# cloudflare/zkp-ecdsa

Measured on NVIDIA H100. Metric: ZKAttest proofs/sec, higher is better.
Workload: dtype u256/u258 (32-bit limbs, Montgomery)

## Files before the change

### zkp_ecdsa_b200/csrc/zk_ops.cuh

```cuda
#pragma once
#include "zk_curves.cuh"
#include "zk_layout.h"
#include "zk_sha256.cuh"

namespace zk {

#if defined(__CUDA_ARCH__)
#define ZK_SET_STATUS(ptr, code) atomicCAS((int*)(ptr), 0, (int)(code))
#define ZK_SET_STATUS_OVER(ptr, code, over) \
  do {                                      \
    atomicCAS((int*)(ptr), 0, (int)(code)); \
    atomicCAS((int*)(ptr), (int)(over), (int)(code)); \
  } while (0)
#else
#define ZK_SET_STATUS_OVER(ptr, code, over)              \
  do {                                                   \
    if (*(ptr) == 0 || *(ptr) == (over)) *(ptr) = (code); \
  } while (0)
#define ZK_SET_STATUS(ptr, code) \
  do {                           \
    if (*(ptr) == 0) *(ptr) = (code); \
  } while (0)
#endif

template <int N>
ZK_HD void ld(uint32_t* r, const uint32_t* p) {
#pragma unroll
  for (int i = 0; i < N; i++) r[i] = p[i];
}
template <int N>
ZK_HD void st(uint32_t* p, const uint32_t* r) {
#pragma unroll
  for (int i = 0; i < N; i++) p[i] = r[i];
}

enum : int {
  P256_PROJ_WORDS = 24,
  P256_AFF_WORDS = 16,
#if defined(ZKA_PG_WAR256)
  TOM_PROJ_WORDS = 24,
  TOM_E2_WORDS = 24,
  TOM_AFF_WORDS = 16,
  TOM_PRE_WORDS = 16,
#else
  TOM_PROJ_WORDS = 28,
  TOM_E2_WORDS = 36,
  TOM_AFF_WORDS = 18,
  TOM_PRE_WORDS = 32,
#endif
  NORM_CHUNK_MAX = 64,
};


#if defined(ZKA_PG_WAR256)
ZK_HD void tom_st_xyz(uint32_t* m, const uint32_t* x, const uint32_t* y, const uint32_t* z) {
  st<8>(m, x); st<8>(m + 8, y); st<8>(m + 16, z);
}
ZK_HD void tom_ld_xyz(uint32_t* x, uint32_t* y, uint32_t* z, const uint32_t* m) {
  ld<8>(x, m); ld<8>(y, m + 8); ld<8>(z, m + 16);
}
ZK_HD void tom_ld_pre(TomPre& q, const uint32_t* m) { ld<8>(q.x, m); ld<8>(q.y, m + 8); }
#else
ZK_HD void tom_st_xyz(uint32_t* m, const uint32_t* x, const uint32_t* y, const uint32_t* z) {
  uint32_t w[28];
#pragma unroll
  for (int i = 0; i < 9; i++) { w[i] = x[i]; w[9 + i] = y[i]; w[18 + i] = z[i]; }
  w[27] = 0;
#if defined(__CUDA_ARCH__)
  uint4* v = reinterpret_cast<uint4*>(m);
#pragma unroll
  for (int i = 0; i < 7; i++) v[i] = make_uint4(w[4 * i], w[4 * i + 1], w[4 * i + 2], w[4 * i + 3]);
#else
  for (int i = 0; i < 28; i++) m[i] = w[i];
#endif
}
ZK_HD void tom_ld_xyz(uint32_t* x, uint32_t* y, uint32_t* z, const uint32_t* m) {
  uint32_t w[28];
#if defined(__CUDA_ARCH__)
  const uint4* v = reinterpret_cast<const uint4*>(m);
#pragma unroll
  for (int i = 0; i < 7; i++) {
    const uint4 u = v[i];
    w[4 * i] = u.x; w[4 * i + 1] = u.y; w[4 * i + 2] = u.z; w[4 * i + 3] = u.w;
  }
#else
  for (int i = 0; i < 28; i++) w[i] = m[i];
#endif
#pragma unroll
  for (int i = 0; i < 9; i++) { x[i] = w[i]; y[i] = w[9 + i]; z[i] = w[18 + i]; }
}
ZK_HD void tom_st_efgh(uint32_t* m, const TomEfgh& p) {
  uint32_t w[36];
#pragma unroll
  for (int i = 0; i < 9; i++) { w[i] = p.e[i]; w[9 + i] = p.f[i]; w[18 + i] = p.g[i]; w[27 + i] = p.h[i]; }
#if defined(__CUDA_ARCH__)
  uint4* v = reinterpret_cast<uint4*>(m);
#pragma unroll
  for (int i = 0; i < 9; i++) v[i] = make_uint4(w[4 * i], w[4 * i + 1], w[4 * i + 2], w[4 * i + 3]);
#else
  for (int i = 0; i < 36; i++) m[i] = w[i];
#endif
}
ZK_HD void tom_ld_efgh(uint32_t* e, uint32_t* f, uint32_t* g, uint32_t* h, const uint32_t* m) {
  uint32_t w[36];
#if defined(__CUDA_ARCH__)
  const uint4* v = reinterpret_cast<const uint4*>(m);
#pragma unroll
  for (int i = 0; i < 9; i++) {
    const uint4 u = v[i];
    w[4 * i] = u.x; w[4 * i + 1] = u.y; w[4 * i + 2] = u.z; w[4 * i + 3] = u.w;
  }
#else
  for (int i = 0; i < 36; i++) w[i] = m[i];
#endif
#pragma unroll
  for (int i = 0; i < 9; i++) { e[i] = w[i]; f[i] = w[9 + i]; g[i] = w[18 + i]; h[i] = w[27 + i]; }
}

ZK_HD void tom2_pre_neg(TomPre& q, bool neg) {
  uint32_t nk[9];
  Tomp::neg(nk, q.k);
#pragma unroll
  for (int i = 0; i < 9; i++) {
    const uint32_t a = q.x[i], b = q.y[i];
    q.x[i] = neg ? b : a;
    q.y[i] = neg ? a : b;
    q.k[i] = neg ? nk[i] : q.k[i];
  }
}
ZK_HD void tom_ld_pre(TomPre& q, const uint32_t* m) {
#if defined(__CUDA_ARCH__)
  const uint4* v = reinterpret_cast<const uint4*>(m);
  uint32_t w[32];
#pragma unroll
  for (int i = 0; i < 7; i++) {
    uint4 u = __ldg(v + i);
    w[4 * i] = u.x; w[4 * i + 1] = u.y; w[4 * i + 2] = u.z; w[4 * i + 3] = u.w;
  }
#pragma unroll
  for (int i = 0; i < 9; i++) { q.x[i] = w[i]; q.y[i] = w[9 + i]; q.k[i] = w[18 + i]; }
#else
  ld<9>(q.x, m); ld<9>(q.y, m + 9); ld<9>(q.k, m + 18);
#endif
}

#endif

ZK_HD void ld4(uint32_t* w, const void* p) {
#if defined(__CUDA_ARCH__)
  const uint4 u = *reinterpret_cast<const uint4*>(p);
  w[0] = u.x; w[1] = u.y; w[2] = u.z; w[3] = u.w;
#else
  const uint32_t* q = reinterpret_cast<const uint32_t*>(p);
  for (int i = 0; i < 4; i++) w[i] = q[i];
#endif
}
ZK_HD void st4(void* p, const uint32_t* w) {
#if defined(__CUDA_ARCH__)
  *reinterpret_cast<uint4*>(p) = make_uint4(w[0], w[1], w[2], w[3]);
#else
  uint32_t* q = reinterpret_cast<uint32_t*>(p);
  for (int i = 0; i < 4; i++) q[i] = w[i];
#endif
}
ZK_HD void ld8v(uint32_t* r, const uint32_t* p) { ld4(r, p); ld4(r + 4, p + 4); }
ZK_HD void st8v(uint32_t* p, const uint32_t* r) { st4(p, r); st4(p + 4, r + 4); }
ZK_HD bool aligned16(const void* p) { return ((size_t)p & 15) == 0; }

template <int N, int CB>
// ... 245 lines not shown
      const uint32_t* src = proj + (size_t)(lo + k) * TOM_PROJ_WORDS;
      uint32_t xx[9];
      tom_ld_xyz(xx, y, z, src);
      F::mul(den, y, z);
      F::mul(acc, acc, den);
      copy_n<9>(pf[k], acc);
    }
    uint32_t inv[9], s2[9], dd2[9];
    F::inv(inv, acc);
    tom_const(s2, TOM_SQRTND1);
    tom_const(dd2, TOM_2D2);
    for (int k = n - 1; k >= 0; k--) {
      const uint32_t* src = proj + (size_t)(lo + k) * TOM_PROJ_WORDS;
      uint32_t x[9], di[9], w[9], v[9], kk[9], ym[9], yp[9];
      tom_ld_xyz(x, y, z, src);
      F::mul(den, y, z);
      if (k > 0) F::mul(di, inv, pf[k - 1]); else copy_n<9>(di, inv);
      F::mul(inv, inv, den);
      F::mul(w, x, y);
      F::mul(w, w, di);
      F::mul(w, w, s2);
      F::sqr(v, z);
      F::mul(v, v, di);
      F::mul(kk, w, v);
      F::mul(kk, kk, dd2);
      F::sub(ym, v, w);
      F::add(yp, v, w);
      F::reduce(ym); F::reduce(yp); F::reduce(kk);
      uint32_t* o = pre + (size_t)(lo + k) * TOM_PRE_WORDS;
      st<9>(o, ym); st<9>(o + 9, yp); st<9>(o + 18, kk);
      for (int i = 27; i < 32; i++) o[i] = 0;
    }
  }
};

struct TomNormTask {
  const uint32_t* proj;
  uint32_t* aff;
  uint8_t* bytes;
  int count;
  int chunk;
  int e2;
  int aff_mod, aff_lim;
  int stride;
  ZK_HD static void canon2p(uint32_t* r) {
    uint32_t t[9], p2[9];
#pragma unroll
    for (int i = 0; i < 9; i++) p2[i] = (FpTom::p(i) << 1) | (i > 0 ? (FpTom::p(i - 1) >> 31) : 0u);
    uint32_t br = sub_n<9>(t, r, p2);
    csel_n<9>(r, br == 0, t, r);
    br = sub_p<FpTom>(t, r);
    csel_n<9>(r, br == 0, t, r);
  }
  ZK_HD void operator()(int t) const {
    using F = Tomp;
    const int lo = t * chunk;
    int n = count - lo;
    if (n > chunk) n = chunk;
    if (n <= 0) return;
    uint32_t pre[NORM_CHUNK_MAX][9];
    uint32_t acc[9], z[9], h[9], den[9];
    F::set_one(acc);
    for (int k = 0; k < n; k++) {
      const uint32_t* src = proj + (size_t)(lo + k) * stride;
      uint32_t xx[9], yy[9];
      if (e2) {
        tom_ld_efgh(xx, yy, z, h, src);
        F::mul(den, z, h);
      } else {
        tom_ld_xyz(xx, yy, den, src);
      }
      F::mul(acc, acc, den);
      copy_n<9>(pre[k], acc);
    }
    uint32_t inv[9], cxk[9], is2[9], one_plain[9];
    F::inv(inv, acc);
    tom_const(cxk, e2 ? TOM_INVSQRTND : TOM_INVSQRTA);
    tom_const(is2, TOM_INVSQRTND1);
    zero_n<9>(one_plain);
    one_plain[0] = 1;
    for (int k = n - 1; k >= 0; k--) {
      const uint32_t* src = proj + (size_t)(lo + k) * stride;
      uint32_t X[9], Y[9], di[9];
      if (e2) {
        tom_ld_efgh(X, Y, z, h, src);
        F::mul(den, z, h);
        F::mul(X, X, h);
        F::mul(Y, Y, z);
      } else {
        tom_ld_xyz(X, Y, den, src);
      }
      if (k > 0) F::mul(di, inv, pre[k - 1]); else copy_n<9>(di, inv);
      F::mul(inv, inv, den);
      if (bytes) {
        uint32_t Dp[9], cx[9], cy[9];
        F::mul(Dp, di, one_plain);
        F::mul(cx, X, cxk);
        F::mul(cx, cx, Dp);
        F::mul(cy, Y, Dp);
        canon2p(cx);
        canon2p(cy);
        store_point_words<9, 33>(bytes + (size_t)(lo + k) * BSTRIDE, 0x04u, cx, cy);
      }
      if (aff && ((lo + k) % aff_mod) < aff_lim) {
        uint32_t x[9], y[9];
        F::mul(x, X, di);
        if (e2) F::mul(x, x, is2);
        F::mul(y, Y, di);
        uint32_t* a = aff + (size_t)(lo + k) * TOM_AFF_WORDS;
        st<9>(a, x);
        st<9>(a + 9, y);
      }
    }
  }
};

ZK_HD void tom2_ld_entry(TomPre& q, const uint32_t* tab, int j, size_t ne, uint32_t d, bool neg) {
  tom_ld_pre(q, tab + ((size_t)j * ne + d) * TOM_PRE_WORDS);
  tom2_pre_neg(q, neg);
}

struct TomCommitTask {
  const uint32_t* jv;
  const uint32_t* jr;
  const uint32_t* gtab;
  const uint32_t* htab;
  uint32_t* proj;
  int w, nwin;
  int xyz = 0;
  ZK_HD void operator()(int t) const {
    uint32_t v[8], r[8];
    ld<8>(v, jv + (size_t)t * 8);
    ld<8>(r, jr + (size_t)t * 8);
    const size_t ne = (size_t)fb_entries(w);
    uint32_t cv = 0, cr = 0;
    bool nv, nr;
    TomPre q;
    uint32_t dv = signed_digit(v, 0, w, cv, nv);
    tom2_ld_entry(q, gtab, 0, ne, dv, nv);
    TomPt acc;
    tom2_from_pre(acc, q);
    for (int j = 0;; j++) {
      const uint32_t dr = signed_digit(r, j, w, cr, nr);
      tom2_ld_entry(q, htab, j, ne, dr, nr);
      if (j == nwin - 1) break;
      tom2_madd<true>(acc, acc, q);
      dv = signed_digit(v, j + 1, w, cv, nv);
      tom2_ld_entry(q, gtab, j + 1, ne, dv, nv);
      tom2_madd<true>(acc, acc, q);
    }
    if (xyz) {
      tom2_madd<false>(acc, acc, q);
      tom_st_xyz(proj + (size_t)t * TOM_PROJ_WORDS, acc.x, acc.y, acc.z);
    } else {
      TomEfgh e;
      tom2_madd_end(e, acc, q);
      tom_st_efgh(proj + (size_t)t * TOM_E2_WORDS, e);
    }
  }
};

struct TomCommitGTask {
// ... 259 lines not shown
```

### zkp_ecdsa_b200/csrc/zk_ops_war.cuh

```cuda
#pragma once

#define WEI_PT WarPt
#define WEI_AFF WarAff
#define WEI_JAC WarJac
#define WEI_F Warp
#define WEI_FN(n) war_##n
#define WEI_T(n) War##n
#include "zk_weier_ops.inc"
#undef WEI_PT
#undef WEI_AFF
#undef WEI_JAC
#undef WEI_F
#undef WEI_FN
#undef WEI_T

struct TomNormTask {
  const uint32_t* proj;
  uint32_t* aff;
  uint8_t* bytes;
  int count;
  int chunk;
  int e2;
  int aff_mod, aff_lim;
  int stride;
  ZK_HD void operator()(int t) const {
    using F = Warp;
    const int lo = t * chunk;
    int n = count - lo;
    if (n > chunk) n = chunk;
    if (n <= 0) return;
    uint32_t pre[NORM_CHUNK_MAX][8];
    uint32_t acc[8], z[8], one[8];
    F::set_one(one);
    copy_n<8>(acc, one);
    for (int k = 0; k < n; k++) {
      ld<8>(z, proj + (size_t)(lo + k) * stride + 16);
      if (is_zero_n<8>(z)) copy_n<8>(z, one);
      F::mul(acc, acc, z);
      copy_n<8>(pre[k], acc);
    }
    uint32_t inv[8];
    F::inv(inv, acc);
    for (int k = n - 1; k >= 0; k--) {
      const uint32_t* src = proj + (size_t)(lo + k) * stride;
      ld<8>(z, src + 16);
      const bool isinf = is_zero_n<8>(z);
      if (isinf) copy_n<8>(z, one);
      uint32_t zi[8];
      if (k > 0) F::mul(zi, inv, pre[k - 1]); else copy_n<8>(zi, inv);
      F::mul(inv, inv, z);
      uint32_t X[8], Y[8], x[8], y[8];
      ld<8>(X, src);
      ld<8>(Y, src + 8);
      F::mul(x, X, zi);
      F::mul(y, Y, zi);
      if (aff && ((lo + k) % aff_mod) < aff_lim) {
        uint32_t* a = aff + (size_t)(lo + k) * TOM_AFF_WORDS;
        st<8>(a, x);
        st<8>(a + 8, y);
      }
      if (bytes) {
        uint32_t cx[8], cy[8];
        F::from_mont(cx, x);
        F::from_mont(cy, y);
        if (isinf) { zero_n<8>(cx); zero_n<8>(cy); }
        store_point_words<8, 32>(bytes + (size_t)(lo + k) * BSTRIDE, isinf ? 0x00u : 0x04u, cx, cy);
      }
    }
  }
};

struct TomCommitTask {
  const uint32_t* jv;
  const uint32_t* jr;
  const uint32_t* gtab;
  const uint32_t* htab;
  uint32_t* proj;
  int w, nwin;
  int xyz = 0;
  ZK_HD void operator()(int t) const {
    uint32_t v[8], r[8];
    ld<8>(v, jv + (size_t)t * 8);
    ld<8>(r, jr + (size_t)t * 8);
    WarJac aj;
    war_set_identity_jac(aj);
    war_accum_fixed_jac(aj, gtab, v, w);
    war_accum_fixed_jac(aj, htab, r, w);
    WarPt acc;
    war_jac_to_hom(acc, aj);
    war_st_proj(proj + (size_t)t * TOM_PROJ_WORDS, acc);
  }
};
struct TomCommitGTask {
  const uint32_t* jv;
  const uint32_t* gtab;
  uint32_t* ext;
  int w, nwin;
  ZK_HD void operator()(int t) const {
    const int item = t / GJOBS_PER_ITEM, g = t % GJOBS_PER_ITEM;
    uint32_t v[8];
    ld<8>(v, jv + ((size_t)item * JOBS_PER_ITEM + item_job_of_gpart(g)) * 8);
    WarJac aj;
    war_set_identity_jac(aj);
    war_accum_fixed_jac(aj, gtab, v, w);
    WarPt acc;
    war_jac_to_hom(acc, aj);
    war_st_proj(ext + (size_t)t * TOM_EXT_WORDS, acc);
  }
};
struct TomCommitHTask {
  const uint32_t* jr;
  const uint32_t* htab;
  const uint32_t* ext;
  uint32_t* proj;
  int w, nwin;
  ZK_HD void operator()(int t) const {
    const int item = t / JOBS_PER_ITEM, jb = t % JOBS_PER_ITEM;
    uint32_t r[8];
    ld<8>(r, jr + (size_t)t * 8);
// ... 7 lines not shown
```

### zkp_ecdsa_b200/csrc/zk_weier_ops.inc

```
ZK_HD void WEI_FN(ld_proj)(WEI_PT& p, const uint32_t* m) {
  ld<8>(p.x, m); ld<8>(p.y, m + 8); ld<8>(p.z, m + 16);
}
ZK_HD void WEI_FN(st_proj)(uint32_t* m, const WEI_PT& p) {
  st<8>(m, p.x); st<8>(m + 8, p.y); st<8>(m + 16, p.z);
}
ZK_HD void WEI_FN(ld_aff)(WEI_AFF& a, const uint32_t* m) { ld<8>(a.x, m); ld<8>(a.y, m + 8); }
ZK_HD void WEI_FN(st_aff)(uint32_t* m, const WEI_AFF& a) { st<8>(m, a.x); st<8>(m + 8, a.y); }

struct WEI_T(PowsTask) {
  const uint32_t* base_aff;
  const uint8_t* base_inf;
  uint32_t* pows;
  int nbase, nwin, w;
  const uint32_t* index = nullptr;
  const uint32_t* count_dev = nullptr;
  const uint32_t* w_dev = nullptr;
  ZK_HD void operator()(int t) const {
    if (count_dev && (uint32_t)t >= *count_dev) return;
    const int w = w_dev ? (int)*w_dev : this->w;
    const int nwin = w_dev ? fb_windows(w) : this->nwin;
    const size_t src = index ? index[t] : (size_t)t;
    WEI_AFF a;
    WEI_FN(ld_aff)(a, base_aff + src * P256_AFF_WORDS);
    WEI_PT p;
// ... 56 lines not shown
      WEI_FN(st_proj)(out + (size_t)(blk * 16 + i) * P256_PROJ_WORDS, acc);
    }
  }
};
struct WEI_T(RowsHiTask) {
  const uint32_t* pows;
  uint32_t* hi;
  uint32_t* rows;
  int w;
  ZK_HD void operator()(int t) const {
    WEI_PT p, acc;
    WEI_FN(ld_proj)(p, pows + (size_t)t * P256_PROJ_WORDS);
    for (int k = 0; k < 8; k++) WEI_FN(dbl)(p, p);
    WEI_FN(set_identity)(acc);
    const int nh = 1 << (w - 9);
    for (int m = 0; m < nh; m++) {
      WEI_FN(st_proj)(hi + ((size_t)t * nh + m) * P256_PROJ_WORDS, acc);
      WEI_FN(add)(acc, acc, p);
    }
    WEI_FN(st_proj)(rows + ((size_t)t * fb_entries(w) + ((size_t)1 << (w - 1))) * P256_PROJ_WORDS, acc);
  }
};
struct WEI_T(RowsLoTask) {
  const uint32_t* pows;
  const uint32_t* hi;
  uint32_t* rows;
  int w;
  ZK_HD void operator()(int t) const {
    const int nh = 1 << (w - 9);
    const int j = t / nh, m = t % nh;
    WEI_PT p, acc;
    WEI_FN(ld_proj)(p, pows + (size_t)j * P256_PROJ_WORDS);
    WEI_FN(ld_proj)(acc, hi + (size_t)t * P256_PROJ_WORDS);
    uint32_t* out = rows + ((size_t)j * fb_entries(w) + ((size_t)m << 8)) * P256_PROJ_WORDS;
    for (int d = 0; d < 256; d++) {
      WEI_FN(st_proj)(out + (size_t)d * P256_PROJ_WORDS, acc);
      WEI_FN(add)(acc, acc, p);
    }
  }
};

struct WEI_T(NormTask) {
  const uint32_t* proj;
  uint32_t* aff;
  uint8_t* bytes;
  uint8_t* inf;
  int count;
  int chunk;
  const uint32_t* groups_dev = nullptr;
  int group_size = 0;
  const uint32_t* w_dev = nullptr;
  ZK_HD void operator()(int t) const {
    using F = WEI_F;
    const int lo = t * chunk;
    int total = count;
    const int group_size = w_dev ? fb_windows((int)*w_dev) * fb_entries((int)*w_dev) : this->group_size;
    if (groups_dev) {
      const long long present = (long long)*groups_dev * group_size;
      if (present < total) total = (int)present;
    }
    int n = total - lo;
    if (n > chunk) n = chunk;
    if (n <= 0) return;
    uint32_t pre[NORM_CHUNK_MAX][8];
    uint32_t acc[8], z[8], one[8];
    F::set_one(one);
    copy_n<8>(acc, one);
    for (int k = 0; k < n; k++) {
      ld<8>(z, proj + (size_t)(lo + k) * P256_PROJ_WORDS + 16);
      if (is_zero_n<8>(z)) copy_n<8>(z, one);
      F::mul(acc, acc, z);
      copy_n<8>(pre[k], acc);
    }
    uint32_t inv[8];
    F::inv(inv, acc);
    for (int k = n - 1; k >= 0; k--) {
      const uint32_t* src = proj + (size_t)(lo + k) * P256_PROJ_WORDS;
      ld<8>(z, src + 16);
      const bool isinf = is_zero_n<8>(z);
      if (isinf) copy_n<8>(z, one);
      uint32_t zi[8];
      if (k > 0) F::mul(zi, inv, pre[k - 1]); else copy_n<8>(zi, inv);
      F::mul(inv, inv, z);
      WEI_AFF a;
      uint32_t X[8], Y[8];
      ld<8>(X, src);
      ld<8>(Y, src + 8);
      F::mul(a.x, X, zi);
      F::mul(a.y, Y, zi);
      WEI_FN(st_aff)(aff + (size_t)(lo + k) * P256_AFF_WORDS, a);
      if (inf) inf[lo + k] = isinf ? 1 : 0;
      if (bytes) {
        uint8_t* o = bytes + (size_t)(lo + k) * BSTRIDE;
        uint32_t cx[8], cy[8];
        F::from_mont(cx, a.x);
        F::from_mont(cy, a.y);
        if (isinf) { zero_n<8>(cx); zero_n<8>(cy); }
        store_point_words<8, 32>(o, isinf ? 0x00u : 0x04u, cx, cy);
      }
    }
  }
};

ZK_HD void WEI_FN(accum_fixed_jac)(WEI_JAC& acc, const uint32_t* tab, const uint32_t* k, int w) {
  const int nwin = fb_windows(w);
  const size_t E = (size_t)fb_entries(w);
  uint32_t carry = 0;
  for (int j = 0; j < nwin; j++) {
    bool neg;
    const uint32_t d = signed_digit(k, j, w, carry, neg);
    if (d) {
      WEI_AFF q;
      WEI_FN(ld_aff)(q, tab + ((size_t)j * E + d) * P256_AFF_WORDS);
      if (neg) WEI_F::neg(q.y, q.y);
      WEI_FN(jac_madd)(acc, acc, q);
    }
  }
}
ZK_HD void WEI_FN(accum_fixed)(WEI_PT& acc, const uint32_t* tab, const uint32_t* k, int w) {
  WEI_JAC q;
  WEI_FN(hom_to_jac)(q, acc);
  WEI_FN(accum_fixed_jac)(q, tab, k, w);
  WEI_FN(jac_to_hom)(acc, q);
}
ZK_HD void WEI_FN(set_identity_jac)(WEI_JAC& p) {
  WEI_F::set_one(p.x);
  WEI_F::set_one(p.y);
  zero_n<8>(p.z);
}
```

### zkp_ecdsa_b200/csrc/zkattest.cu

```cuda
#include "zkattest.h"

#include <math.h>
#include <stdio.h>

#include <algorithm>
#include <atomic>
#include <cmath>
#include <mutex>
#include <chrono>
#include <memory>
#include <thread>
#include <string>
#include <vector>

#include "zk_launch.cuh"
#include "zk_prove.cuh"
#include "zk_seed.cuh"
#include "zk_verify_agg.cuh"

namespace zk {
struct ParsePointsTask {
  const uint8_t* nist;
  const uint8_t* tom;
  uint32_t* nist_aff;
// ... 314 lines not shown
namespace {

int fail(zka_ctx* ctx, int code, const std::string& msg) {
  if (ctx) ctx->err = msg;
  return code;
}
template <class Fn>
int guarded(zka_ctx* ctx, Fn&& body) {
  try {
    return body();
  } catch (const std::exception& e) {
    return fail(ctx, ZKA_E_CUDA, e.what());
  }
}

template <class Src>
void agg_msm(Stream& st, Cursor A, const Src& src, const AggPlan& pl, const uint32_t* ctl, const uint32_t** rootA,
             const uint32_t** rootB) {
  const AggDigits& D = pl.D;
  const int nwin = D.nwin, nb = D.nb, nseg = (nb + 1 + AGG_SEG - 1) / AGG_SEG;
  const size_t cap = (size_t)src.slots();
  uint32_t* hist = A.take<uint32_t>((size_t)nwin * (nb + 1));
  uint32_t* bstart = A.take<uint32_t>((size_t)nwin * (nb + 2));
  uint32_t* segtot = A.take<uint32_t>((size_t)nwin * nseg);
  uint32_t* sorted = A.take<uint32_t>((size_t)nwin * cap);
  uint32_t* bsum = A.take<uint32_t>((size_t)nwin * nb * Src::PTW);
  dev_memset(st, hist, 0, (size_t)nwin * (nb + 1) * 4);
  launch(st, (long long)cap, AggHistTask<Src>{src, D, ctl, hist});
  launch(st, (long long)nwin * nseg, AggSegSumTask{ctl, hist, segtot, nb, nseg});
  launch(st, nwin, AggSegScanTask{ctl, segtot, nseg});
  launch(st, (long long)nwin * nseg, AggOffsetsTask{ctl, segtot, hist, bstart, nb, nseg});
  launch(st, (long long)cap, AggScatterTask<Src>{src, D, ctl, hist, sorted, cap});
  launch(st, (long long)nwin * nb, AggBucketTask<Src>{src, ctl, bstart, sorted, bsum, cap, nb});
  const uint32_t *inA = bsum, *inB = nullptr;
  int nin = nb, ll = 0;
  for (int lv = 0; lv < pl.levels; lv++) {
    const int nout = nin >> pl.lm[lv];
    uint32_t* oA = A.take<uint32_t>((size_t)nwin * nout * Src::PTW);
    uint32_t* oB = A.take<uint32_t>((size_t)nwin * nout * Src::PTW);
    launch(st, (long long)nwin * nout, AggLevelTask<Src>{ctl, inA, inB, oA, oB, nin, pl.lm[lv], ll, nwin, D.top_shift});
    inA = oA; inB = oB; nin = nout; ll += pl.lm[lv];
  }
  *rootA = inA;
  *rootB = inB;
}

int ceil_log2(uint32_t v) {
  int n = 0;
  while ((1ull << n) < v) n++;
  return n;
}


static int g_norm_slots = 132 * 4;
static bool g_norm_model = true;
inline int norm_chunk_for(long long count, int per_point = 11) {
  if (!g_norm_model) {
    long long c = count / 100000;
    if (c < 8) c = 8;
    if (c > NORM_CHUNK_MAX) c = NORM_CHUNK_MAX;
    return (int)c;
  }
  int best = 8;
  long long best_cost = -1;
  for (int c = 8; c <= NORM_CHUNK_MAX; c++) {
    const long long threads = (count + c - 1) / c, ctas = (threads + 127) / 128;
    const long long waves = (ctas + g_norm_slots - 1) / g_norm_slots;
    const long long cost = waves * ((long long)per_point * c + 70);
    if (best_cost < 0 || cost < best_cost) { best_cost = cost; best = c; }
  }
  return best;
}
inline void launch_p256_norm(Stream& st, const uint32_t* proj, uint32_t* aff, uint8_t* bytes, uint8_t* inf, long long count) {
  if (count <= 0) return;
  const int ch = norm_chunk_for(count, bytes ? 7 : 5);
  launch(st, (count + ch - 1) / ch, P256NormTask{proj, aff, bytes, inf, (int)count, ch});
}
inline void launch_tom_norm(Stream& st, const uint32_t* proj, uint32_t* aff, uint8_t* bytes, long long count, int e2,
                            int aff_mod = 1, int aff_lim = 1, int stride = 0) {
  if (count <= 0) return;
  const int ch = norm_chunk_for(count);
  if (stride == 0) stride = e2 ? TOM_E2_WORDS : TOM_PROJ_WORDS;
  launch(st, (count + ch - 1) / ch, TomNormTask{proj, aff, bytes, (int)count, ch, e2, aff_mod, aff_lim, stride});
}

void build_p256_tab(zka_ctx* ctx, const uint32_t* base_aff_dev, FixedTable& out, int w) {
  Stream& st = ctx->st;
  const int nwin = fb_windows(w);
  const size_t E = (size_t)fb_entries(w), count = (size_t)nwin * E;
  DevBuf pows, rows;
  uint32_t* d_pows = pows.get<uint32_t>((size_t)nwin * P256_PROJ_WORDS);
  uint32_t* d_rows = rows.get<uint32_t>(count * P256_PROJ_WORDS);
  out.tab = out.buf.get<uint32_t>(count * P256_AFF_WORDS);
  launch(st, 1, P256PowsTask{base_aff_dev, nullptr, d_pows, 1, nwin, w});
  if (w > 9) {
    DevBuf hi;
    const int nh = 1 << (w - 9);
    uint32_t* d_hi = hi.get<uint32_t>((size_t)nwin * nh * P256_PROJ_WORDS);
    launch(st, nwin, P256RowsHiTask{d_pows, d_hi, d_rows, w});
    launch(st, (long long)nwin * nh, P256RowsLoTask{d_pows, d_hi, d_rows, w});
    sync(st);
  } else {
    launch(st, nwin, P256RowsTask{d_pows, d_rows, w});
  }
  launch_p256_norm(st, d_rows, out.tab, nullptr, nullptr, (long long)(count));
  sync(st);
}
#if defined(ZKA_PG_WAR256)
void build_tom_tab(zka_ctx* ctx, const uint32_t* base_aff_dev, FixedTable& out) {
  Stream& st = ctx->st;
  const int w = ctx->tom_w, nwin = fb_windows(w);
  const size_t E = (size_t)fb_entries(w), count = (size_t)nwin * E;
  DevBuf pows, rows;
  uint32_t* d_pows = pows.get<uint32_t>((size_t)nwin * P256_PROJ_WORDS);
  uint32_t* d_rows = rows.get<uint32_t>(count * P256_PROJ_WORDS);
  out.tab = out.buf.get<uint32_t>(count * TOM_PRE_WORDS);
  launch(st, 1, WarPowsTask{base_aff_dev, nullptr, d_pows, 1, nwin, w});
  if (w > 9) {
    DevBuf hi;
    const int nh = 1 << (w - 9);
    uint32_t* d_hi = hi.get<uint32_t>((size_t)nwin * nh * P256_PROJ_WORDS);
    launch(st, nwin, WarRowsHiTask{d_pows, d_hi, d_rows, w});
    launch(st, (long long)nwin * nh, WarRowsLoTask{d_pows, d_hi, d_rows, w});
    sync(st);
  } else {
    launch(st, nwin, WarRowsTask{d_pows, d_rows, w});
  }
  {
    const int ch = norm_chunk_for((long long)count, 5);
    launch(st, ((long long)count + ch - 1) / ch, WarNormTask{d_rows, out.tab, nullptr, nullptr, (int)count, ch});
  }
  sync(st);
}
#else
void build_tom_tab(zka_ctx* ctx, const uint32_t* base_aff_dev, FixedTable& out) {
  Stream& st = ctx->st;
  const int w = ctx->tom_w, nwin = ctx->tom_nwin;
  const size_t ne = (size_t)fb_entries(w), count = (size_t)nwin * ne;
  DevBuf pows, rows;
  uint32_t* d_pows = pows.get<uint32_t>((size_t)nwin * 36);
  uint32_t* d_rows = rows.get<uint32_t>(count * TOM_PROJ_WORDS);
  out.tab = out.buf.get<uint32_t>(count * TOM_PRE_WORDS);
  launch(st, 1, TomPowsTask{base_aff_dev, d_pows, 1, nwin, w});
  if (w > 9) {
    DevBuf hi;
    const int nh = 1 << (w - 9);
    uint32_t* d_hi = hi.get<uint32_t>((size_t)nwin * nh * 36);
    launch(st, nwin, TomRowsHiTask{d_pows, d_hi, d_rows, w});
    launch(st, (long long)nwin * nh, TomRowsLoTask{d_pows, d_hi, d_rows, w});
    sync(st);
  } else {
    launch(st, nwin, TomRowsTask{d_pows, d_rows, w});
  }
  launch(st, (long long)(count + 15) / 16, TomTabE2Task{d_rows, out.tab, (int)count});
  sync(st);
}

#endif

template <class T>
const T* stage_in(Stream& st, DevBuf& buf, const T* p, size_t count) {
  if (!p || count == 0) return p;
  if (is_device_ptr(p)) return p;
  T* d = buf.get<T>(count);
  copy_h2d(st, d, p, count * sizeof(T));
  return d;
}

template <class T>
struct Output {
  T* dst;
  size_t width;
  bool dev;
  Output(T* p, size_t width) : dst(p), width(width), dev(is_device_ptr(p)) {}
  T* rows(DevBuf& stage, uint32_t b0, size_t rows) const { return dev ? dst + b0 * width : stage.get<T>(rows * width); }
  void copy_back(Stream& st, uint32_t b0, const T* d, size_t rows) const {
    if (!dev) copy_d2h(st, dst + b0 * width, d, rows * width * sizeof(T));
  }
  void copy_back_2d(Stream& st, uint32_t b0, const T* d, size_t rows, size_t bytes) const {
    if (!dev) copy_d2h_2d(st, dst + b0 * width, width * sizeof(T), d, width * sizeof(T), bytes, rows);
  }
};

// ... 290 lines not shown
  return 0;
}
int zka_set_progress(zka_ctx* ctx, volatile uint32_t* flags, uint32_t cap) {
  if (!ctx) return ZKA_E_ARG;
  ctx->progress = flags;
  ctx->progress_cap = flags ? cap : 0;
  return 0;
}
int zka_chunk_schedule(zka_ctx* ctx, uint32_t B, int host_buffers, uint32_t* off, uint32_t cap) {
  if (!ctx || !off || cap == 0) return ZKA_E_ARG;
  const std::vector<uint32_t> v = chunk_schedule(B, (uint32_t)(host_buffers ? std::min(ctx->chunk, ctx->host_chunk) : ctx->chunk), ctx->nlanes,
                                                 host_buffers != 0);
  if (v.size() > cap) return ZKA_E_ARG;
  for (size_t i = 0; i < v.size(); i++) off[i] = v[i];
  return (int)v.size() - 1;
}
int zka_lanes(const zka_ctx* ctx) { return ctx ? ctx->nlanes : 0; }
int zka_config(const zka_ctx* ctx, int* tom_w, int* tom_nwin, int* chunk) {
  if (!ctx) return ZKA_E_ARG;
  if (tom_w) *tom_w = ctx->tom_w;
  if (tom_nwin) *tom_nwin = ctx->tom_nwin;
  if (chunk) *chunk = ctx->chunk;
  return 0;
}

int zka_init(int device, zka_ctx** out) {
  if (!out) return ZKA_E_ARG;
  *out = nullptr;
#if !defined(ZKA_HOSTSIM)
  int ndev = 0;
  cudaError_t e = cudaGetDeviceCount(&ndev);
  if (e != cudaSuccess || ndev == 0 || device >= ndev) {
    cudaGetLastError();
    return ZKA_E_CUDA;
  }
#endif
  std::unique_ptr<zka_ctx> ctx(new zka_ctx());
  const int rc = guarded(ctx.get(), [&] {
#if !defined(ZKA_HOSTSIM)
    ZK_CUDA_CHECK(cudaSetDevice(device));
    ZK_CUDA_CHECK(cudaStreamCreateWithFlags(&ctx->st.s, cudaStreamNonBlocking));
#endif
    ctx->device = device;
    if (const char* e = getenv("ZKA_TOM_W")) {
      int w = atoi(e);
      if (w >= 2 && w <= 24) ctx->tom_w = w;
    }
    ctx->tom_nwin = fb_windows(ctx->tom_w);
    if (const char* e = getenv("ZKA_CHUNK")) {
      int c = atoi(e);
      if (c >= 1) ctx->chunk = c;
    }
    if (const char* e = getenv("ZKA_NORM_MODEL")) g_norm_model = atoi(e) != 0;
#if !defined(ZKA_HOSTSIM)
    {
      int sms = 0;
      if (cudaDeviceGetAttribute(&sms, cudaDevAttrMultiProcessorCount, device) == cudaSuccess && sms > 0) g_norm_slots = sms * 4;
    }
#endif
    if (const char* e = getenv("ZKA_HOST_CHUNK")) {
      int c = atoi(e);
      if (c >= 1) ctx->host_chunk = c;
    }
    stream_create(ctx->cs_in);
    stream_create(ctx->cs_out);
    stream_create(ctx->aux[0]);
    stream_create(ctx->aux[1]);
    {
      int lanes = 3;
#if defined(ZKA_HOSTSIM)
      lanes = 1;
#endif
      if (const char* e = getenv("ZKA_LANES")) lanes = atoi(e);
      if (lanes < 1) lanes = 1;
      if (lanes > 8) lanes = 8;
      if (zka_set_option(ctx.get(), "lanes", lanes) != 0) throw std::runtime_error("lanes");
    }
    if (const char* e = getenv("ZKA_TAPE_SPLIT")) ctx->tape_split = atoi(e) != 0;
    if (const char* e = getenv("ZKA_AGG")) ctx->agg = atoi(e);
    if (const char* e = getenv("ZKA_AGG_C")) {
      int c = atoi(e);
      if (c >= 4 && c <= 16) ctx->agg_c = c;
    }
    if (const char* e = getenv("ZKA_P256_HW")) {
      int w = atoi(e);
      if (w >= 8 && w <= 24) ctx->p256_hw = w;
    }
    DevBuf gen;
    uint32_t* d_gen = gen.get<uint32_t>(16 + TOM_AFF_WORDS);
    launch(ctx->st, 1, GenAffTask{d_gen, d_gen + 16});
    build_p256_tab(ctx.get(), d_gen, ctx->g8, 8);
    build_p256_tab(ctx.get(), d_gen, ctx->gw, ctx->p256_hw);
    build_tom_tab(ctx.get(), d_gen + 16, ctx->tg);
    DevBuf proj, aff;
    uint32_t* d_proj = proj.get<uint32_t>(TOM_PROJ_WORDS);
    uint32_t* d_aff = aff.get<uint32_t>(TOM_AFF_WORDS);
    uint8_t* d_bytes = ctx->tg_bytes.get<uint8_t>(BSTRIDE);
    launch(ctx->st, 1, GProjTask{d_gen + 16, d_proj});
    launch_tom_norm(ctx->st, d_proj, d_aff, d_bytes, 1, 0);
    sync(ctx->st);
    return 0;
  });
  if (rc) {
    fprintf(stderr, "zka_init: %s\n", ctx->err.c_str());
    return rc;
  }
  *out = ctx.release();
  return 0;
}

// ... 347 lines not shown
        c.q_inf = w.take<uint8_t>(Bc);
        c.r_aff = w.take<uint32_t>((size_t)Bc * 16);
        c.r_bytes = w.take<uint8_t>((size_t)Bc * BSTRIDE);
        c.rpows = w.take<uint32_t>((size_t)Bc * RT_NWIN * P256_PROJ_WORDS);
        c.rrows = w.take<uint32_t>((size_t)Bc * KEY_CAP * P256_PROJ_WORDS);
        c.rtab = w.take<uint32_t>((size_t)Bc * KEY_CAP * P256_AFF_WORDS);
        c.pa_T = w.take<uint32_t>(nA * P256_PROJ_WORDS);
        c.pa_A = w.take<uint32_t>(nA * P256_PROJ_WORDS);
        c.pa_T_aff = w.take<uint32_t>(nA * 16);
        c.pa_T_inf = w.take<uint8_t>(nA);
        c.pa_A_aff = w.take<uint32_t>(nA * 16);
        c.pa_A_bytes = w.take<uint8_t>(nA * BSTRIDE);
        c.pa_A_inf = w.take<uint8_t>(nA);
        c.s1_jv = w.take<uint32_t>(n1 * 8);
        c.s1_jr = w.take<uint32_t>(n1 * 8);
        c.s1_proj = w.take<uint32_t>(n1 * TOM_E2_WORDS);
        c.s1_aff = w.take<uint32_t>(n1 * TOM_AFF_WORDS);
        c.s1_bytes = w.take<uint8_t>(n1 * BSTRIDE);
        c.chal = w.take<uint32_t>((size_t)Bc * 3);
        c.zcount = w.take<uint32_t>(Bc);
        c.item_base = w.take<uint32_t>(Bc);
        c.item_total = w.take<uint32_t>(2);
        c.rep_off = w.take<uint32_t>((size_t)Bc * S);
        c.gk_off = w.take<uint32_t>(Bc);
        c.gk_dv = w.take<uint32_t>((size_t)Bc * n * 8);
        c.gk_x = w.take<uint32_t>((size_t)Bc * 3);
        c.u12 = w.take<uint32_t>((size_t)Bc * 16);
        c.tab_of = w.take<uint32_t>(Bc);
        c.tab_rep = w.take<uint32_t>((size_t)Bc * 2);
        c.tab_count = w.take<uint32_t>(2);
        c.which_s = w.take<uint32_t>(Bc);
        uint32_t* base_aff = w.take_if<uint32_t>(mode == 1, (size_t)Bc * 16);
        c.base_aff = mode == 0 ? c.pk_aff : base_aff;
        c.proof_stride = proof_stride;
        Cursor ob(ln.out[slot]);
        c.proofs = po.rows(ob.next(), b0, Bc);
        c.proof_len = lo.rows(ob.next(), b0, Bc);
        c.status = so.rows(ob.next(), b0, Bc);
  
        launch(st, Bc, PreKeyTask{c});
        launch(st, Bc, KeyDedupTask{c});
        launch(st, Bc, KeyRankTask{c});
        launch(st, Bc, KeyAssignTask{c});
        {
          const int Bp = (Bc + 31) & ~31;
          launch(st, (long long)Bp + Bc,
                 PowsAndPreTask{P256PowsTask{c.base_aff, nullptr, c.rpows, Bc, RT_NWIN, RT_W, c.tab_rep, c.tab_count, c.tab_count + 1}, PreTask{c}, Bp});
        }
        launch(st, (long long)Bc * ((KEY_CAP + 15) / 16), P256RowsBlockTask{c.rpows, c.rrows, KEY_W_MIN, c.tab_count, c.tab_count + 1});
        {
          const long long np = (long long)Bc * KEY_CAP;
          const uint32_t kest = rp ? (uint32_t)Bc : std::min<uint32_t>(N, (uint32_t)Bc);
          const int west = key_window_bits(kest, (uint32_t)Bc, (uint32_t)S + 2);
          const int ch = norm_chunk_for((long long)kest * fb_windows(west) * fb_entries(west), 5);
          launch(st, (np + ch - 1) / ch, P256NormTask{c.rrows, c.rtab, nullptr, nullptr, (int)np, ch, c.tab_count, 0, c.tab_count + 1});
        }
        ev_wait(st, ln.ev_tape[slot]);
        if (seeded) {
          const int d1 = draws_before_items(S);
          launch(st, (long long)Bc * d1, SeedProveTapeTask{cin[slot].seeds, const_cast<uint8_t*>(c.tape), c.tape_stride, S, n, 0, d1, nullptr});
        }
        {
          const int nAp = (int)((nA + 31) & ~(size_t)31);
          launch(st, (long long)nAp + Bc, PhaseAAndRPointTask{PhaseAP256Task{c}, RPointTask{c}, (int)nA, nAp});
        }
        launch_p256_norm(st, c.pa_T, c.pa_T_aff, nullptr, c.pa_T_inf, (long long)(nA));
        launch_p256_norm(st, c.pa_A, c.pa_A_aff, c.pa_A_bytes, c.pa_A_inf, (long long)(nA));
        if (mode == 1) launch(st, Bc, ExpStatementTask{c});
        prove_store1(st, c);
        launch(st, Bc, ExpChallengeTask{c});
        launch(st, 1, ScanTask{c});
        uint32_t tot2[2] = {0, 0};
        copy_d2h(st, tot2, c.item_total, 8);
        const bool tape_host = !seeded && ctx->tape_split && !is_device_ptr(tape);
        sync(st);
        if (seeded) {
          const int d1 = draws_before_items(S), span = prove_draws((int)tot2[1], n, S) - d1;
          launch(st, (long long)Bc * span, SeedProveTapeTask{cin[slot].seeds, const_cast<uint8_t*>(c.tape), c.tape_stride, S, n, d1, span, c.zcount});
        } else if (tape_host) {
          const size_t o0 = (size_t)32 * draws_before_items(S);
          const size_t o1 = std::min(tape_stride, (size_t)32 * prove_draws((int)tot2[1], n, S));
          if (o1 > o0)
            copy_d2h_2d(st, const_cast<uint8_t*>(c.tape) + o0, c.tape_stride, tape + (size_t)b0 * tape_stride + o0, tape_stride, o1 - o0, Bc);
        }
        const double t_mid = ms_now();
        {
          const uint32_t kn = next_chunk.fetch_add(1);
          if (kn < nchunks) issue_inputs(kn, slot ^ 1);
          k = kn;
        }
        const uint32_t M = tot2[0];
        const size_t max_len = mode == 0 ? (size_t)proof_len((int)tot2[1], n, S)
                                         : (size_t)tot2[1] * REP0_LEN + (size_t)(S - (int)tot2[1]) * REP1_LEN;
        c.M = (int)M;
        c.item_b = w.take<uint32_t>(M);
        c.item_i = w.take<uint32_t>(M);
        c.item_k = w.take<uint32_t>(M);
        c.pb_T1 = w.take<uint32_t>((size_t)M * P256_PROJ_WORDS);
        c.pb_T1_aff = w.take<uint32_t>((size_t)M * 16);
        c.pb_T1_inf = w.take<uint8_t>(M);
        const size_t n2 = c.s2_count();
        c.s2_jv = w.take<uint32_t>(n2 * 8);
        c.s2_jr = w.take<uint32_t>(n2 * 8);
        c.s2_proj = w.take<uint32_t>(n2 * TOM_E2_WORDS);
        c.s2_aff = w.take<uint32_t>(n2 * TOM_AFF_WORDS);
        c.s2_bytes = w.take<uint8_t>(n2 * BSTRIDE);
        c.secrets = w.take<uint32_t>((size_t)M * SECRETS_PER_ITEM * 8);
        c.item_inv = w.take<uint32_t>((size_t)M * 8);
// ... 846 lines not shown
```

Measured before the change: 111,900.

## Interleave batch-normalization chunks across warp lanes and prefetch next points

Normalization tasks now assign each thread a strided set of points (stride 32) so lanes in a warp read adjacent points, making global loads coalesced instead of each thread walking a contiguous chunk. The backward pass software-prefetches the next point while processing the current one. The Tom kernel caches the z*h product from the forward pass and folds the one_plain multiplication into the inverse once rather than per point. The chunk model now queries real occupancy per task type and accepts an env override. The changes raise register/local memory use (an extra gh array) and alter the thread-count formula.

```diff
diff --git a/zkp_ecdsa_b200/csrc/zk_ops.cuh b/zkp_ecdsa_b200/csrc/zk_ops.cuh
--- a/zkp_ecdsa_b200/csrc/zk_ops.cuh
+++ b/zkp_ecdsa_b200/csrc/zk_ops.cuh
@@ -51,6 +51,14 @@
   NORM_CHUNK_MAX = 64,
 };
 
+ZK_HD int norm_tile(int t, int chunk, int total, int& first) {
+  first = (t >> 5) * 32 * chunk + (t & 31);
+  if (first >= total) return 0;
+  const int n = (total - first + 31) >> 5;
+  return n < chunk ? n : chunk;
+}
+inline long long norm_threads(long long count, int chunk) { return (count + 32LL * chunk - 1) / (32LL * chunk) * 32; }
+
 
 #if defined(ZKA_PG_WAR256)
 ZK_HD void tom_st_xyz(uint32_t* m, const uint32_t* x, const uint32_t* y, const uint32_t* z) {
@@ -115,6 +123,19 @@
 #endif
 #pragma unroll
   for (int i = 0; i < 9; i++) { e[i] = w[i]; f[i] = w[9 + i]; g[i] = w[18 + i]; h[i] = w[27 + i]; }
+}
+template <int Q>
+ZK_HD void tom_ld_from16(uint32_t* r, const uint32_t* m) {
+#if defined(__CUDA_ARCH__)
+  const uint4* v = reinterpret_cast<const uint4*>(m) + 4;
+#pragma unroll
+  for (int i = 0; i < Q; i++) {
+    const uint4 u = v[i];
+    r[4 * i] = u.x; r[4 * i + 1] = u.y; r[4 * i + 2] = u.z; r[4 * i + 3] = u.w;
+  }
+#else
+  for (int i = 0; i < 4 * Q; i++) r[i] = m[16 + i];
+#endif
 }
 
 ZK_HD void tom2_pre_neg(TomPre& q, bool neg) {
@@ -466,62 +487,78 @@
     br = sub_p<FpTom>(t, r);
     csel_n<9>(r, br == 0, t, r);
   }
+  ZK_HD void ld_slot(uint32_t* a, uint32_t* b, uint32_t* c, uint32_t* d, const uint32_t* src) const {
+    if (e2) tom_ld_efgh(a, b, c, d, src);
+    else tom_ld_xyz(a, b, c, src);
+  }
   ZK_HD void operator()(int t) const {
     using F = Tomp;
-    const int lo = t * chunk;
-    int n = count - lo;
-    if (n > chunk) n = chunk;
-    if (n <= 0) return;
+    int lo;
+    const int n = norm_tile(t, chunk, count, lo);
+    if (n == 0) return;
     uint32_t pre[NORM_CHUNK_MAX][9];
-    uint32_t acc[9], z[9], h[9], den[9];
+    uint32_t gh[NORM_CHUNK_MAX][9];
+    uint32_t acc[9], den[9];
     F::set_one(acc);
     for (int k = 0; k < n; k++) {
-      const uint32_t* src = proj + (size_t)(lo + k) * stride;
-      uint32_t xx[9], yy[9];
+      const uint32_t* src = proj + (size_t)(lo + 32 * k) * stride;
+      uint32_t w[20];
       if (e2) {
-        tom_ld_efgh(xx, yy, z, h, src);
-        F::mul(den, z, h);
+        tom_ld_from16<5>(w, src);
+        F::mul(den, w + 2, w + 11);
+        copy_n<9>(gh[k], den);
       } else {
-        tom_ld_xyz(xx, yy, den, src);
+        tom_ld_from16<3>(w, src);
+        copy_n<9>(den, w + 2);
       }
       F::mul(acc, acc, den);
       copy_n<9>(pre[k], acc);
     }
-    uint32_t inv[9], cxk[9], is2[9], one_plain[9];
+    uint32_t inv[9], cxk[9], is2[9], rr[9];
     F::inv(inv, acc);
+    if (bytes) {
+      uint32_t one_plain[9];
+      zero_n<9>(one_plain);
+      one_plain[0] = 1;
+      F::mul(inv, inv, one_plain);
+    }
     tom_const(cxk, e2 ? TOM_INVSQRTND : TOM_INVSQRTA);
     tom_const(is2, TOM_INVSQRTND1);
-    zero_n<9>(one_plain);
-    one_plain[0] = 1;
+#pragma unroll
+    for (int j = 0; j < 9; j++) rr[j] = FpTom::rr(j);
+    uint32_t nX[9], nY[9], nz[9], nh[9];
+    zero_n<9>(nh);
+    ld_slot(nX, nY, nz, nh, proj + (size_t)(lo + 32 * (n - 1)) * stride);
     for (int k = n - 1; k >= 0; k--) {
-      const uint32_t* src = proj + (size_t)(lo + k) * stride;
-      uint32_t X[9], Y[9], di[9];
+      const int i = lo + 32 * k;
+      uint32_t X[9], Y[9], z[9], h[9], di[9];
+      copy_n<9>(X, nX); copy_n<9>(Y, nY); copy_n<9>(z, nz); copy_n<9>(h, nh);
+      if (k > 0) ld_slot(nX, nY, nz, nh, proj + (size_t)(i - 32) * stride);
       if (e2) {
-        tom_ld_efgh(X, Y, z, h, src);
-        F::mul(den, z, h);
+        copy_n<9>(den, gh[k]);
         F::mul(X, X, h);
         F::mul(Y, Y, z);
       } else {
-        tom_ld_xyz(X, Y, den, src);
+        copy_n<9>(den, z);
       }
       if (k > 0) F::mul(di, inv, pre[k - 1]); else copy_n<9>(di, inv);
       F::mul(inv, inv, den);
       if (bytes) {
-        uint32_t Dp[9], cx[9], cy[9];
-        F::mul(Dp, di, one_plain);
+        uint32_t cx[9], cy[9];
         F::mul(cx, X, cxk);
-        F::mul(cx, cx, Dp);
-        F::mul(cy, Y, Dp);
+        F::mul(cx, cx, di);
+        F::mul(cy, Y, di);
         canon2p(cx);
         canon2p(cy);
-        store_point_words<9, 33>(bytes + (size_t)(lo + k) * BSTRIDE, 0x04u, cx, cy);
+        store_point_words<9, 33>(bytes + (size_t)i * BSTRIDE, 0x04u, cx, cy);
       }
-      if (aff && ((lo + k) % aff_mod) < aff_lim) {
+      if (aff && (i % aff_mod) < aff_lim) {
         uint32_t x[9], y[9];
+        if (bytes) F::mul(di, di, rr);
         F::mul(x, X, di);
         if (e2) F::mul(x, x, is2);
         F::mul(y, Y, di);
-        uint32_t* a = aff + (size_t)(lo + k) * TOM_AFF_WORDS;
+        uint32_t* a = aff + (size_t)i * TOM_AFF_WORDS;
         st<9>(a, x);
         st<9>(a + 9, y);
       }
diff --git a/zkp_ecdsa_b200/csrc/zk_ops_war.cuh b/zkp_ecdsa_b200/csrc/zk_ops_war.cuh
--- a/zkp_ecdsa_b200/csrc/zk_ops_war.cuh
+++ b/zkp_ecdsa_b200/csrc/zk_ops_war.cuh
@@ -25,16 +25,15 @@
   int stride;
   ZK_HD void operator()(int t) const {
     using F = Warp;
-    const int lo = t * chunk;
-    int n = count - lo;
-    if (n > chunk) n = chunk;
-    if (n <= 0) return;
+    int lo;
+    const int n = norm_tile(t, chunk, count, lo);
+    if (n == 0) return;
     uint32_t pre[NORM_CHUNK_MAX][8];
     uint32_t acc[8], z[8], one[8];
     F::set_one(one);
     copy_n<8>(acc, one);
     for (int k = 0; k < n; k++) {
-      ld<8>(z, proj + (size_t)(lo + k) * stride + 16);
+      ld<8>(z, proj + (size_t)(lo + 32 * k) * stride + 16);
       if (is_zero_n<8>(z)) copy_n<8>(z, one);
       F::mul(acc, acc, z);
       copy_n<8>(pre[k], acc);
@@ -42,7 +41,8 @@
     uint32_t inv[8];
     F::inv(inv, acc);
     for (int k = n - 1; k >= 0; k--) {
-      const uint32_t* src = proj + (size_t)(lo + k) * stride;
+      const int i = lo + 32 * k;
+      const uint32_t* src = proj + (size_t)i * stride;
       ld<8>(z, src + 16);
       const bool isinf = is_zero_n<8>(z);
       if (isinf) copy_n<8>(z, one);
@@ -54,8 +54,8 @@
       ld<8>(Y, src + 8);
       F::mul(x, X, zi);
       F::mul(y, Y, zi);
-      if (aff && ((lo + k) % aff_mod) < aff_lim) {
-        uint32_t* a = aff + (size_t)(lo + k) * TOM_AFF_WORDS;
+      if (aff && (i % aff_mod) < aff_lim) {
+        uint32_t* a = aff + (size_t)i * TOM_AFF_WORDS;
         st<8>(a, x);
         st<8>(a + 8, y);
       }
@@ -64,7 +64,7 @@
         F::from_mont(cx, x);
         F::from_mont(cy, y);
         if (isinf) { zero_n<8>(cx); zero_n<8>(cy); }
-        store_point_words<8, 32>(bytes + (size_t)(lo + k) * BSTRIDE, isinf ? 0x00u : 0x04u, cx, cy);
+        store_point_words<8, 32>(bytes + (size_t)i * BSTRIDE, isinf ? 0x00u : 0x04u, cx, cy);
       }
     }
   }
diff --git a/zkp_ecdsa_b200/csrc/zk_weier_ops.inc b/zkp_ecdsa_b200/csrc/zk_weier_ops.inc
--- a/zkp_ecdsa_b200/csrc/zk_weier_ops.inc
+++ b/zkp_ecdsa_b200/csrc/zk_weier_ops.inc
@@ -132,46 +132,52 @@
   const uint32_t* w_dev = nullptr;
   ZK_HD void operator()(int t) const {
     using F = WEI_F;
-    const int lo = t * chunk;
     int total = count;
     const int group_size = w_dev ? fb_windows((int)*w_dev) * fb_entries((int)*w_dev) : this->group_size;
     if (groups_dev) {
       const long long present = (long long)*groups_dev * group_size;
       if (present < total) total = (int)present;
     }
-    int n = total - lo;
-    if (n > chunk) n = chunk;
-    if (n <= 0) return;
+    int lo;
+    const int n = norm_tile(t, chunk, total, lo);
+    if (n == 0) return;
     uint32_t pre[NORM_CHUNK_MAX][8];
     uint32_t acc[8], z[8], one[8];
     F::set_one(one);
     copy_n<8>(acc, one);
     for (int k = 0; k < n; k++) {
-      ld<8>(z, proj + (size_t)(lo + k) * P256_PROJ_WORDS + 16);
+      ld<8>(z, proj + (size_t)(lo + 32 * k) * P256_PROJ_WORDS + 16);
       if (is_zero_n<8>(z)) copy_n<8>(z, one);
       F::mul(acc, acc, z);
       copy_n<8>(pre[k], acc);
     }
     uint32_t inv[8];
     F::inv(inv, acc);
+    uint32_t nX[8], nY[8], nz[8];
+    {
+      const uint32_t* src = proj + (size_t)(lo + 32 * (n - 1)) * P256_PROJ_WORDS;
+      ld<8>(nX, src); ld<8>(nY, src + 8); ld<8>(nz, src + 16);
+    }
     for (int k = n - 1; k >= 0; k--) {
-      const uint32_t* src = proj + (size_t)(lo + k) * P256_PROJ_WORDS;
-      ld<8>(z, src + 16);
+      const int i = lo + 32 * k;
+      uint32_t X[8], Y[8];
+      copy_n<8>(X, nX); copy_n<8>(Y, nY); copy_n<8>(z, nz);
+      if (k > 0) {
+        const uint32_t* src = proj + (size_t)(i - 32) * P256_PROJ_WORDS;
+        ld<8>(nX, src); ld<8>(nY, src + 8); ld<8>(nz, src + 16);
+      }
       const bool isinf = is_zero_n<8>(z);
       if (isinf) copy_n<8>(z, one);
       uint32_t zi[8];
       if (k > 0) F::mul(zi, inv, pre[k - 1]); else copy_n<8>(zi, inv);
       F::mul(inv, inv, z);
       WEI_AFF a;
-      uint32_t X[8], Y[8];
-      ld<8>(X, src);
-      ld<8>(Y, src + 8);
       F::mul(a.x, X, zi);
       F::mul(a.y, Y, zi);
-      WEI_FN(st_aff)(aff + (size_t)(lo + k) * P256_AFF_WORDS, a);
-      if (inf) inf[lo + k] = isinf ? 1 : 0;
+      WEI_FN(st_aff)(aff + (size_t)i * P256_AFF_WORDS, a);
+      if (inf) inf[i] = isinf ? 1 : 0;
       if (bytes) {
-        uint8_t* o = bytes + (size_t)(lo + k) * BSTRIDE;
+        uint8_t* o = bytes + (size_t)i * BSTRIDE;
         uint32_t cx[8], cy[8];
         F::from_mont(cx, a.x);
         F::from_mont(cy, a.y);
diff --git a/zkp_ecdsa_b200/csrc/zkattest.cu b/zkp_ecdsa_b200/csrc/zkattest.cu
--- a/zkp_ecdsa_b200/csrc/zkattest.cu
+++ b/zkp_ecdsa_b200/csrc/zkattest.cu
@@ -390,36 +390,52 @@
 }
 
 
-static int g_norm_slots = 132 * 4;
+constexpr int NORM_INV_COST = 70;
+static int g_norm_sms = 132;
 static bool g_norm_model = true;
+static int g_norm_chunk = 0;
+template <class Task>
+int norm_slots() {
+  static int per_sm = 0;
+#if !defined(ZKA_HOSTSIM)
+  if (per_sm == 0 && cudaOccupancyMaxActiveBlocksPerMultiprocessor(&per_sm, zk_task_kernel<Task>, 128, 0) != cudaSuccess) {
+    cudaGetLastError();
+    per_sm = 0;
+  }
+#endif
+  return g_norm_sms * (per_sm > 0 ? per_sm : 4);
+}
+template <class Task>
 inline int norm_chunk_for(long long count, int per_point = 11) {
+  if (g_norm_chunk) return g_norm_chunk;
   if (!g_norm_model) {
     long long c = count / 100000;
     if (c < 8) c = 8;
     if (c > NORM_CHUNK_MAX) c = NORM_CHUNK_MAX;
     return (int)c;
   }
+  const int slots = norm_slots<Task>();
   int best = 8;
   long long best_cost = -1;
   for (int c = 8; c <= NORM_CHUNK_MAX; c++) {
-    const long long threads = (count + c - 1) / c, ctas = (threads + 127) / 128;
-    const long long waves = (ctas + g_norm_slots - 1) / g_norm_slots;
-    const long long cost = waves * ((long long)per_point * c + 70);
+    const long long ctas = (norm_threads(count, c) + 127) / 128;
+    const long long waves = (ctas + slots - 1) / slots;
+    const long long cost = waves * ((long long)per_point * c + NORM_INV_COST);
     if (best_cost < 0 || cost < best_cost) { best_cost = cost; best = c; }
   }
   return best;
 }
 inline void launch_p256_norm(Stream& st, const uint32_t* proj, uint32_t* aff, uint8_t* bytes, uint8_t* inf, long long count) {
   if (count <= 0) return;
-  const int ch = norm_chunk_for(count, bytes ? 7 : 5);
-  launch(st, (count + ch - 1) / ch, P256NormTask{proj, aff, bytes, inf, (int)count, ch});
+  const int ch = norm_chunk_for<P256NormTask>(count, bytes ? 7 : 5);
+  launch(st, norm_threads(count, ch), P256NormTask{proj, aff, bytes, inf, (int)count, ch});
 }
 inline void launch_tom_norm(Stream& st, const uint32_t* proj, uint32_t* aff, uint8_t* bytes, long long count, int e2,
                             int aff_mod = 1, int aff_lim = 1, int stride = 0) {
   if (count <= 0) return;
-  const int ch = norm_chunk_for(count);
+  const int ch = norm_chunk_for<TomNormTask>(count);
   if (stride == 0) stride = e2 ? TOM_E2_WORDS : TOM_PROJ_WORDS;
-  launch(st, (count + ch - 1) / ch, TomNormTask{proj, aff, bytes, (int)count, ch, e2, aff_mod, aff_lim, stride});
+  launch(st, norm_threads(count, ch), TomNormTask{proj, aff, bytes, (int)count, ch, e2, aff_mod, aff_lim, stride});
 }
 
 void build_p256_tab(zka_ctx* ctx, const uint32_t* base_aff_dev, FixedTable& out, int w) {
@@ -465,8 +481,8 @@
     launch(st, nwin, WarRowsTask{d_pows, d_rows, w});
   }
   {
-    const int ch = norm_chunk_for((long long)count, 5);
-    launch(st, ((long long)count + ch - 1) / ch, WarNormTask{d_rows, out.tab, nullptr, nullptr, (int)count, ch});
+    const int ch = norm_chunk_for<WarNormTask>((long long)count, 5);
+    launch(st, norm_threads((long long)count, ch), WarNormTask{d_rows, out.tab, nullptr, nullptr, (int)count, ch});
   }
   sync(st);
 }
@@ -863,10 +879,14 @@
       if (c >= 1) ctx->chunk = c;
     }
     if (const char* e = getenv("ZKA_NORM_MODEL")) g_norm_model = atoi(e) != 0;
+    if (const char* e = getenv("ZKA_NORM_CHUNK")) {
+      int c = atoi(e);
+      if (c >= 1 && c <= NORM_CHUNK_MAX) g_norm_chunk = c;
+    }
 #if !defined(ZKA_HOSTSIM)
     {
       int sms = 0;
-      if (cudaDeviceGetAttribute(&sms, cudaDevAttrMultiProcessorCount, device) == cudaSuccess && sms > 0) g_norm_slots = sms * 4;
+      if (cudaDeviceGetAttribute(&sms, cudaDevAttrMultiProcessorCount, device) == cudaSuccess && sms > 0) g_norm_sms = sms;
     }
 #endif
     if (const char* e = getenv("ZKA_HOST_CHUNK")) {
@@ -1320,8 +1340,8 @@
           const long long np = (long long)Bc * KEY_CAP;
           const uint32_t kest = rp ? (uint32_t)Bc : std::min<uint32_t>(N, (uint32_t)Bc);
           const int west = key_window_bits(kest, (uint32_t)Bc, (uint32_t)S + 2);
-          const int ch = norm_chunk_for((long long)kest * fb_windows(west) * fb_entries(west), 5);
-          launch(st, (np + ch - 1) / ch, P256NormTask{c.rrows, c.rtab, nullptr, nullptr, (int)np, ch, c.tab_count, 0, c.tab_count + 1});
+          const int ch = norm_chunk_for<P256NormTask>((long long)kest * fb_windows(west) * fb_entries(west), 5);
+          launch(st, norm_threads(np, ch), P256NormTask{c.rrows, c.rtab, nullptr, nullptr, (int)np, ch, c.tab_count, 0, c.tab_count + 1});
         }
         ev_wait(st, ln.ev_tape[slot]);
         if (seeded) {
```

Result: no change. 112,700 (median of 6 runs) (+0.7%).
